# bittremieux/falcon

Measured on AMD Instinct MI355X. Metric: spectra clustered/sec @1/2/4/8 GPU; cosine-kernel HBM GB/s vs roofline, higher is better.
Workload: dtype f32; 1 GPU; one dataset of 1000000 synthetic spectra (1000000 per GPU; charges 2+3; precursor m/z 400-1200), low_dim=400, n_neighbors=64, n_neighbors_ann=128, n_probe=16, eps=0.1, precursor_tol=20ppm, mz_interval=1.0, batch_size=32768; exchange=none, parallelism=1 GPU

## Files before the change

### falcon_amd/csrc/core.hip

```cpp
#include <math.h>
#include <stdarg.h>
#include <stdlib.h>
#include <string.h>
#include "common.h"
#include "hash.h"
#include "scan.h"
#include "ivf.h"
#include <algorithm>

#include <chrono>
namespace fal {
static bool trace_alloc() {
    static int v = -1;
    if (v < 0) {
        const char* e = getenv("FALCON_TRACE_ALLOC");
        v = e && e[0] && e[0] != '0';
    }
    return v == 1;
}
static hipError_t traced_malloc(void** p, size_t bytes, const char* what, int id) {
    if (!trace_alloc()) return hipMalloc(p, bytes);
    const auto t0 = std::chrono::steady_clock::now();
    const hipError_t e = hipMalloc(p, bytes);
    const double ms = std::chrono::duration<double, std::milli>(std::chrono::steady_clock::now() - t0).count();
// ... 128 lines not shown
    if (!arena) FAL_CHECK_HIP(hipHostMalloc((void**)&arena, kArena, hipHostMallocDefault));
    size_t off = (arena_off + 63) & ~(size_t)63;
    if (off + bytes > kArena) {
        FAL_CHECK_HIP(hipStreamSynchronize(stream));
        off = 0;
    }
    memcpy(arena + off, src, bytes);
    FAL_CHECK_HIP(hipMemcpyAsync(dst, arena + off, bytes, hipMemcpyHostToDevice, stream));
    arena_off = off + bytes;
    return FAL_OK;
}

int fal_ctx::stage_begin(int stage, hipEvent_t* stop_out, hipStream_t on) {
    StageTimer& t = timers[stage];
    if (t.used == t.ev.size()) {
        hipEvent_t a, b;
        FAL_CHECK_HIP(hipEventCreate(&a));
        FAL_CHECK_HIP(hipEventCreate(&b));
        t.ev.push_back({a, b});
    }
    FAL_CHECK_HIP(hipEventRecord(t.ev[t.used].first, on ? on : stream));
    *stop_out = t.ev[t.used].second;
    t.used++;
    return FAL_OK;
}

int fal_ctx::stage_end(hipEvent_t stop, hipStream_t on) {
    FAL_CHECK_HIP(hipEventRecord(stop, on ? on : stream));
    return FAL_OK;
}

extern "C" {

int fal_version(void) { return 100; }

const char* fal_last_error(void) { return fal::g_err; }

int fal_device_count(int* count) {
    FAL_REQUIRE(count, FAL_EINVAL, "fal_device_count: NULL");
    int n = 0;
    hipError_t e = hipGetDeviceCount(&n);
    if (e != hipSuccess) n = 0;
    *count = n;
    return FAL_OK;
}

int fal_ctx_create(int device, void* stream, int own_stream, fal_ctx** out) {
    FAL_REQUIRE(out, FAL_EINVAL, "fal_ctx_create: out is NULL");
    *out = nullptr;
    int n = 0;
    if (hipGetDeviceCount(&n) != hipSuccess || n <= 0) {
        fal::set_error("fal_ctx_create: no HIP device visible (this library has no CPU fallback)");
        return FAL_ENODEV;
    }
    FAL_REQUIRE(device >= 0 && device < n, FAL_EINVAL, "fal_ctx_create: device %d out of range [0,%d)", device, n);
    FAL_CHECK_HIP(hipSetDevice(device));
    hipDeviceProp_t prop;
    FAL_CHECK_HIP(hipGetDeviceProperties(&prop, device));
    if (strncmp(prop.gcnArchName, "gfx950", 6) != 0) {
        fal::set_error("fal_ctx_create: device %d is %s; this library is built for gfx950 only", device, prop.gcnArchName);
        return FAL_ENODEV;
    }
    fal_ctx* c = new fal_ctx();
    c->device = device;
    c->num_cus = prop.multiProcessorCount;
    c->persistent_wgs = c->num_cus;
    if (const char* e = getenv("FALCON_PERSISTENT_WGS")) {
        const int v = atoi(e);
        if (v >= 8 && v <= c->num_cus) c->persistent_wgs = v;
    }
    if (!own_stream) {
        c->stream = (hipStream_t)stream;
        c->own_stream = false;
    } else {
        hipError_t e = hipStreamCreateWithFlags(&c->stream, hipStreamNonBlocking);
        if (e != hipSuccess) {
            delete c;
            fal::set_error("hipStreamCreate failed: %s", hipGetErrorString(e));
            return FAL_EHIP;
        }
        c->own_stream = true;
    }
    if (hipHostMalloc((void**)&c->fb_host, 64, hipHostMallocDefault) != hipSuccess ||
        hipMalloc((void**)&c->zero_dev, 64) != hipSuccess || hipMemset(c->zero_dev, 0, 64) != hipSuccess) {
        fal::set_error("fal_ctx_create: cannot allocate the context's counters");
        fal_ctx_destroy(c);
        return FAL_ENOMEM;
    }
    memset(c->fb_host, 0, 64);
    const char* dbg = getenv("FALCON_DEBUG_POISON");
    c->debug_poison = dbg && dbg[0] && dbg[0] != '0';
    *out = c;
    return FAL_OK;
}

int fal_ctx_destroy(fal_ctx* c) {
    if (!c) return FAL_OK;
    (void)hipSetDevice(c->device);
    (void)hipStreamSynchronize(c->stream);
    for (auto& s : c->scratch)
        if (s.ptr) (void)hipFree(s.ptr);
    for (void* p : c->retired) (void)hipFree(p);
    for (auto& b : c->pool) (void)hipFree(b.ptr);
    if (c->pinned) (void)hipHostFree(c->pinned);
    if (c->fb_host) (void)hipHostFree(c->fb_host);
    if (c->zero_dev) (void)hipFree(c->zero_dev);
    if (c->arena) (void)hipHostFree(c->arena);
    for (auto& t : c->timers)
        for (auto& p : t.ev) {
            (void)hipEventDestroy(p.first);
            (void)hipEventDestroy(p.second);
        }
    if (c->own_stream) (void)hipStreamDestroy(c->stream);
    delete c;
    return FAL_OK;
}

int fal_ctx_plan(fal_ctx* c, int64_t n, int low_dim, int k_ann, int n_probe, int64_t batch_size) {
    fal::CallScope _call(c);
    FAL_REQUIRE(c && n >= 0 && low_dim >= 1 && k_ann >= 1 && n_probe >= 1 && batch_size >= 1, FAL_EINVAL, "fal_ctx_plan: bad argument");
    FAL_CHECK_HIP(hipSetDevice(c->device));
    for (const void* k : fal::warm_kernels()) {
        hipFuncAttributes attr;
        FAL_CHECK_HIP(hipFuncGetAttributes(&attr, k));
    }
    if (!c->arena) FAL_CHECK_HIP(hipHostMalloc((void**)&c->arena, (size_t)32u << 20, hipHostMallocDefault));
    if (n == 0) return FAL_OK;
    void* p = nullptr;
    using namespace fal;
    const size_t nn = (size_t)n;
    FAL_TRY(c->reserve(SLOT_SORT, 24 * nn + 4096, &p));
    FAL_TRY(c->reserve(SLOT_SORT2, 12 * nn + 4096, &p));
    {
        const char* e = getenv("FALCON_SIMS_MB");
        size_t cap = (e ? (size_t)atoll(e) : 2048) * 1024 * 1024;
        const double need = 4.0 * (double)nn * (double)std::min<int64_t>(n, std::min<int64_t>(batch_size, 4096));
        if (need < (double)cap) cap = (size_t)need;
        FAL_TRY(c->reserve(SLOT_SIMS, cap + sizeof(float) * kSimsSlack, &p));
    }
    for (int slot : {SLOT_DB, SLOT_DB2, SLOT_TAIL, SLOT_TAIL2, SLOT_FIN, SLOT_FIN2}) FAL_TRY(c->reserve(slot, 8 * nn + 4096, &p));
    for (int slot = 0; slot < fal::kNumSlots; ++slot) c->release(slot);
    return FAL_OK;
}

int fal_ctx_trim(fal_ctx* c) {
    fal::CallScope _call(c);
    FAL_REQUIRE(c, FAL_EINVAL, "fal_ctx_trim: NULL ctx");
    FAL_CHECK_HIP(hipStreamSynchronize(c->stream));
    c->release_retired();
    for (auto& s : c->scratch)
        if (s.ptr) {
            (void)hipFree(s.ptr);
            s.ptr = nullptr;
            s.cap = 0;
        }
    size_t kept = 0;
    for (size_t i = 0; i < c->pool.size(); ++i) {
        if (c->pool[i].used) c->pool[kept++] = c->pool[i];
        else (void)hipFree(c->pool[i].ptr);
    }
    c->pool.resize(kept);
    return FAL_OK;
}

int fal_ctx_sync(fal_ctx* c) {
    fal::CallScope _call(c);
    FAL_REQUIRE(c, FAL_EINVAL, "fal_ctx_sync: NULL ctx");
    FAL_CHECK_HIP(hipStreamSynchronize(c->stream));
    return FAL_OK;
}

int fal_ctx_enable_timing(fal_ctx* c, int on) {
    FAL_REQUIRE(c, FAL_EINVAL, "NULL ctx");
    c->timing = on != 0;
    return FAL_OK;
}

int fal_ctx_counter(fal_ctx* c, int which, int64_t* value) {
    FAL_REQUIRE(c && value && which >= 0 && which < 10, FAL_EINVAL, "fal_ctx_counter: bad argument");
    *value = c->counters[which];
    if (which == 5) *value = c->fb_host ? (int64_t)c->fb_host[0] + (int64_t)c->fb_host[2] : 0;
    return FAL_OK;
}

int fal_ctx_stage_ms(fal_ctx* c, int stage, float* ms, int64_t* launches) {
    fal::CallScope _call(c);
    FAL_REQUIRE(c && ms && stage >= 0 && stage < fal::kNumStages, FAL_EINVAL, "fal_ctx_stage_ms: bad argument");
    FAL_CHECK_HIP(hipStreamSynchronize(c->stream));
    float total = 0.f;
    auto& t = c->timers[stage];
    for (size_t i = 0; i < t.used; ++i) {
        float x = 0.f;
        FAL_CHECK_HIP(hipEventElapsedTime(&x, t.ev[i].first, t.ev[i].second));
        total += x;
    }
    *ms = total;
    if (launches) *launches = (int64_t)t.used;
    return FAL_OK;
}

int fal_get_dim(float min_mz, float max_mz, float bin_size, uint32_t* dim, float* start_dim, float* end_dim) {
    FAL_REQUIRE(dim && start_dim && end_dim, FAL_EINVAL, "fal_get_dim: NULL output");
    FAL_REQUIRE(bin_size > 0.f && max_mz >= min_mz, FAL_EINVAL, "fal_get_dim: need bin_size > 0 and max_mz >= min_mz");
    volatile float s = min_mz - fmodf(min_mz, bin_size);
    volatile float t = max_mz + bin_size;
    volatile float e = t - fmodf(max_mz, bin_size);
    volatile float w = e - s;
    volatile float q = w / bin_size;
    *start_dim = s;
    *end_dim = e;
    *dim = (uint32_t)ceilf(q);
    return FAL_OK;
}

int fal_hash_lookup(uint32_t n_bins, uint32_t low_dim, uint32_t seed, uint32_t* out_table) {
    FAL_REQUIRE(out_table && low_dim > 0, FAL_EINVAL, "fal_hash_lookup: bad argument");
    for (uint32_t i = 0; i < n_bins; ++i) out_table[i] = fal::murmur3_32(i, seed) % low_dim;
    return FAL_OK;
}

}
```

### falcon_amd/csrc/scan.h

```cpp
#pragma once
#include "common.h"
#include "simtile.h"

namespace fal {

enum { EPI_STORE = 0, EPI_ARGMAX = 1 };
enum { MODE_DENSE = 0, MODE_IVF = 1 };

constexpr size_t kSimsSlack = 2048;

struct SelectArgs {
    const float* sims;
    int64_t sims_base;
    int k;
    float* out_sim;
    int32_t* out_idx;
    const DenseJob* jobs;
    int n_jobs;
    int64_t tile_begin;
    const int32_t* tile_job;
    int ids_are_rows;
    int n_probe;
    const int32_t* probes;
    const int64_t* list_off;
    const int64_t* q_sim_off;
    const int32_t* perm;
    const float* f_pmz;
    const float* f_rt;
    double f_tol, f_rt_tol;
    int f_is_da;
    int f_keep;
    int32_t* nb_idx;
    float* nb_dist;
    int32_t* nb_count;
};

bool dense4_supports(int d);
int launch_dense4(fal_ctx* ctx, const float* X, int d, const DenseJob* jobs, const DenseJob* jobs_host, int n_jobs, float* sims,
                  int64_t sims_base);
bool dense4ab_supports(int d);
int launch_dense4ab(fal_ctx* ctx, const float* X, int d, const DenseJob* jobs, const DenseJob* jobs_host, int n_jobs, float* sims,
                    int64_t sims_base);
int launch_dense_tiny4(fal_ctx* ctx, const float* X, int d, const DenseJob* jobs, int n_jobs, float* sims, int64_t sims_base);
int launch_flat_exact_small(fal_ctx* ctx, const float* X, int d, const DenseJob* jobs, int n_jobs, float* sims, int64_t sims_base);
int launch_dense(fal_ctx* ctx, int stage, int epi, const float* Q, const float* Cm, int d, const DenseJob* jobs,
                 int n_jobs, int64_t tile_begin, int64_t n_tiles, float* sims, int64_t sims_base, int32_t* assign,
                 int64_t xcd_list_tiles = 0);
constexpr int kAssignSeg = 2048;
constexpr int kAssignGroup = 128;
constexpr int kAssignMergeLists = 2048;
struct AssignJob {
    int64_t row0;
    int64_t cent0;
    int32_t nrows;
    int32_t ncent;
    int32_t id_base;
    int32_t part0;
};
int launch_assign(fal_ctx* ctx, int stage, const float* X, const float* centroids, int d, const AssignJob* jobs, int64_t n_jobs,
                  int64_t n_wave_jobs, int64_t n, unsigned long long* keys, int32_t* assign);
bool assign16_supports(int d);
int launch_cvt_f16(fal_ctx* ctx, const float* in, void* out, int64_t count);
int launch_assign16(fal_ctx* ctx, int stage, const void* X16, const float* X, const void* C16, const float* Cn, int d,
                    const AssignJob* jobs, int64_t n_single, int64_t n_merge, int64_t n_group, int64_t n_rows, int32_t* assign,
                    uint16_t* ckeys = nullptr, int ckeys_stride = 0, const uint16_t* sp_cols = nullptr,
                    const float* sp_vals = nullptr, int merge_max_lists = 4 * kAssignGroup, int64_t merge_rows = 0);
struct ListScanArgs {
    const float* Xl;
    int d;
    const int64_t* list_off;
    const int64_t* inv_off;
    const int64_t* ltile_off;
    int group_shift;
    const int32_t* inv_q;
    const int64_t* inv_dest;
    int64_t list_begin, list_end;
    int64_t tile_begin, n_tiles_max;
    float* sims;
    int64_t sims_base;
    float* sink;
};
int launch_list_scan(fal_ctx* ctx, const ListScanArgs& a);
int launch_select(fal_ctx* ctx, int stage, int mode, const SelectArgs& a, int64_t n_blocks, hipStream_t on = nullptr);
int launch_scan16(fal_ctx* ctx, int planes, const void* Xs, int d, const DenseJob* jobs, int n_jobs, int64_t list_tiles,
                  float* sims, int64_t sims_base, float* sink);

}
```

### falcon_amd/csrc/scan.hip

```cpp
#include <math.h>
#include <stdlib.h>
#include <string.h>
#include <algorithm>
#include "common.h"
#include "simtile.h"
#include "scan.h"
#include "select.h"
#include "ivf.h"

namespace fal {

template <int DH4, int EPI>
__global__ __launch_bounds__(64, 1) void dense_kernel(
    const float* __restrict__ Q, const float* __restrict__ Cm, int d, const DenseJob* __restrict__ jobs,
    int n_jobs, int64_t tile_begin, int64_t n_tiles, float* __restrict__ sims, int64_t sims_base,
    int32_t* __restrict__ assign, int xcd_lists, int symmetric) {
    DenseJob job;
    int lt;
    int ji = 0;
    if (xcd_lists) {
        if (!find_job_xcd(jobs, n_jobs, blockIdx.x, &ji, &lt)) return;
        job = jobs[ji];
    } else {
        const int64_t per_xcd = (n_tiles + 7) / 8;
// ... 434 lines not shown
}

int launch_flat_exact_small(fal_ctx* ctx, const float* X, int d, const DenseJob* jobs, int n_jobs, float* sims, int64_t sims_base) {
    if (n_jobs <= 0) return FAL_OK;
    StageScope ts(ctx, ST_SCAN);
    hipLaunchKernelGGL(flat_exact_small_kernel, dim3((unsigned)std::min<int64_t>(n_jobs, (int64_t)ctx->num_cus * 16)), dim3(64), 0,
                       ctx->stream, X, d, jobs, n_jobs, sims, sims_base);
    FAL_CHECK_HIP(hipGetLastError());
    return FAL_OK;
}

int launch_dense_tiny4(fal_ctx* ctx, const float* X, int d, const DenseJob* jobs, int n_jobs, float* sims, int64_t sims_base) {
    if (n_jobs <= 0) return FAL_OK;
    const int dh4 = d / 8;
    const size_t lds = (size_t)2 * 32 * (d * 4 + 16);
    int32_t* cursors = nullptr;
    FAL_TRY(ctx->reserve(SLOT_CURSORS, sizeof(int32_t) * 16, (void**)&cursors));
    cursors += 8;
    dim3 grid((unsigned)std::min<int64_t>(ceil_div(n_jobs, 4), ctx->persistent_wgs)), block(256);
    StageScope ts(ctx, ST_SCAN);
    FAL_CHECK_HIP(hipMemsetAsync(cursors, 0, sizeof(int32_t), ctx->stream));
#define FAL_LAUNCH_TINY4(DH4)                                                                                       \
    do {                                                                                                            \
        FAL_CHECK_HIP(hipFuncSetAttribute((const void*)dense_tiny4_kernel<DH4>, hipFuncAttributeMaxDynamicSharedMemorySize, \
                                          (int)lds));                                                               \
        hipLaunchKernelGGL((dense_tiny4_kernel<DH4>), grid, block, lds, ctx->stream, X, d, jobs, n_jobs, sims, sims_base, \
                           cursors);                                                                                \
    } while (0)
    if (dh4 <= 8) FAL_LAUNCH_TINY4(8);
    else if (dh4 <= 16) FAL_LAUNCH_TINY4(16);
    else if (dh4 <= 32) FAL_LAUNCH_TINY4(32);
    else if (dh4 <= 50) FAL_LAUNCH_TINY4(50);
    else {
        set_error("dense_tiny4 supports low_dim <= 400 (got %d)", d);
        return FAL_EUNSUPPORTED;
    }
#undef FAL_LAUNCH_TINY4
    FAL_CHECK_HIP(hipGetLastError());
    return FAL_OK;
}

template <int EPI>
static int launch_dense_t(fal_ctx* ctx, int stage, const float* Q, const float* Cm, int d, const DenseJob* jobs,
                          int n_jobs, int64_t tile_begin, int64_t n_tiles, float* sims, int64_t sims_base,
                          int32_t* assign, int64_t xcd_list_tiles) {
    if (n_tiles <= 0) return FAL_OK;
    const int symmetric = (EPI == EPI_STORE && xcd_list_tiles > 0 && Q == Cm) ? 1 : 0;
    const int dh4 = d / 8;
    const int xcd_lists = xcd_list_tiles > 0;
    const int64_t per_xcd = xcd_lists ? xcd_list_tiles : (n_tiles + 7) / 8;
    FAL_REQUIRE(per_xcd * 8 < (int64_t)INT32_MAX, FAL_EUNSUPPORTED, "too many tiles in one launch");
 dim3 grid((unsigned)(per_xcd * 8)), block(64);
    StageScope ts(ctx, stage);
    StageScope tk(ctx, ST_KERNEL, nullptr, stage == ST_SCAN);
#define FAL_LAUNCH_DENSE(DH4)                                                                              \
    hipLaunchKernelGGL((dense_kernel<DH4, EPI>), grid, block, 0, ctx->stream, Q, Cm, d, jobs, n_jobs,      \
                       tile_begin, n_tiles, sims, sims_base, assign, xcd_lists, symmetric)
    if (dh4 <= 8) FAL_LAUNCH_DENSE(8);
    else if (dh4 <= 16) FAL_LAUNCH_DENSE(16);
    else if (dh4 <= 32) FAL_LAUNCH_DENSE(32);
    else if (dh4 <= 50) FAL_LAUNCH_DENSE(50);
    else if (dh4 <= 64) FAL_LAUNCH_DENSE(64);
    else {
        set_error("float32 scan supports low_dim <= 512 (got %d)", d);
        return FAL_EUNSUPPORTED;
    }
#undef FAL_LAUNCH_DENSE
    FAL_CHECK_HIP(hipGetLastError());
    return FAL_OK;
}

int launch_dense(fal_ctx* ctx, int stage, int epi, const float* Q, const float* Cm, int d, const DenseJob* jobs,
                 int n_jobs, int64_t tile_begin, int64_t n_tiles, float* sims, int64_t sims_base, int32_t* assign,
                 int64_t xcd_list_tiles) {
    if (epi == EPI_STORE)
        return launch_dense_t<EPI_STORE>(ctx, stage, Q, Cm, d, jobs, n_jobs, tile_begin, n_tiles, sims, sims_base,
                                         assign, xcd_list_tiles);
    return launch_dense_t<EPI_ARGMAX>(ctx, stage, Q, Cm, d, jobs, n_jobs, tile_begin, n_tiles, sims, sims_base, assign,
                                      xcd_list_tiles);
}

template <int MODE, bool FUSE>
__global__ __launch_bounds__(64) __attribute__((amdgpu_waves_per_eu(MODE == MODE_DENSE ? 8 : 3, 8))) void select_kernel(SelectArgs a) {
    __shared__ uint32_t sel_u[kSelBuf];
    __shared__ uint32_t sel_id[kSelBuf];
    __shared__ int64_t seg_off[FAL_MAX_N_PROBE + 1];
    __shared__ int64_t seg_src[FAL_MAX_N_PROBE];
    const int lane = threadIdx.x;
    const int k = a.k;
    const unsigned qblock = blockIdx.x;

    SelQuery qy{nullptr, 0, 0};
    int64_t out_row = 0;
    const int64_t t = a.tile_begin + (qblock >> 5);
    const int ql = qblock & 31;
    const DenseJob job = a.jobs[a.tile_job[qblock >> 5]];
    const int lt = (int)(t - job.tile0);
    if (32 * lt + ql >= job.nq) return;
    if (MODE == MODE_DENSE) {
        qy.nc = job.nc;
        qy.row = a.sims + (job.obase - a.sims_base) + (int64_t)(32 * lt + ql) * ((job.nc + 31) & ~31);
        out_row = job.q_row0 + 32 * (int64_t)lt + ql;
        qy.id0 = a.ids_are_rows ? job.c_row0 : 0;
    } else {
        const int64_t p = job.q_row0 + 32 * (int64_t)lt + ql;
        const int np = a.n_probe;
        const int32_t* pr = a.probes + p * np;
        const int64_t lbase = job.c_row0;
        if (lane == 0) {
            int64_t off = 0;
            for (int j = 0; j < np; ++j) {
                const int32_t l = pr[j];
                seg_off[j] = off;
                if (l >= 0) {
                    const int64_t b = a.list_off[lbase + l], e = a.list_off[lbase + l + 1];
                    seg_src[j] = b;
                    off += e - b;
                } else {
                    seg_src[j] = 0;
                }
            }
            seg_off[np] = off;
        }
        __syncthreads();
        qy.nc = seg_off[np];
        qy.row = a.sims + (a.q_sim_off[32 * t + ql] - a.sims_base);
        out_row = a.perm[p];
    }

    int carry;
    if (qy.nc <= 128) carry = select_rounds<MODE, 2>(a, qy, k, lane, sel_u, sel_id, seg_off, seg_src);
    else if (qy.nc <= 256) carry = select_rounds<MODE, 4>(a, qy, k, lane, sel_u, sel_id, seg_off, seg_src);
    else if (qy.nc <= 384) carry = select_rounds<MODE, 6>(a, qy, k, lane, sel_u, sel_id, seg_off, seg_src);
    else if (qy.nc <= 512) carry = select_rounds<MODE, 8>(a, qy, k, lane, sel_u, sel_id, seg_off, seg_src);
    else if (qy.nc <= 768) carry = select_rounds<MODE, 12>(a, qy, k, lane, sel_u, sel_id, seg_off, seg_src);
    else carry = select_rounds<MODE, 16>(a, qy, k, lane, sel_u, sel_id, seg_off, seg_src);

    if constexpr (FUSE) {
        filter_sort_store(a, sel_u, sel_id, sel_u + FAL_MAX_K_ANN, sel_id + FAL_MAX_K_ANN, carry, out_row, lane);
    } else {
        float* osim = a.out_sim + out_row * k;
        int32_t* oidx = a.out_idx + out_row * k;
        if (k <= 64) sort_and_store<1>(sel_u, sel_id, carry, k, lane, osim, oidx);
        else if (k <= 128) sort_and_store<2>(sel_u, sel_id, carry, k, lane, osim, oidx);
        else sort_and_store<4>(sel_u, sel_id, carry, k, lane, osim, oidx);
    }
}

__global__ void tile_job_kernel(const DenseJob* __restrict__ jobs, int n_jobs, int64_t tile_begin, int64_t n_tiles,
                                int32_t* __restrict__ tile_job) {
    const int64_t i = blockIdx.x * (int64_t)blockDim.x + threadIdx.x;
    if (i < n_tiles) tile_job[i] = find_job(jobs, n_jobs, tile_begin + i);
}

int launch_select(fal_ctx* ctx, int stage, int mode, const SelectArgs& a_in, int64_t n_blocks, hipStream_t on) {
    if (n_blocks <= 0) return FAL_OK;
    SelectArgs a = a_in;
    {
        const int64_t n_tiles = n_blocks / 32;
        int32_t* tj = nullptr;
        ctx->release(SLOT_TILEJOB);
        FAL_TRY(ctx->reserve(SLOT_TILEJOB, sizeof(int32_t) * (size_t)std::max<int64_t>(n_tiles, 1 << 16), (void**)&tj));
        hipLaunchKernelGGL(tile_job_kernel, dim3((unsigned)ceil_div(n_tiles, 256)), dim3(256), 0, on ? on : ctx->stream, a.jobs,
                           a.n_jobs, a.tile_begin, n_tiles, tj);
        a.tile_job = tj;
    }
    FAL_REQUIRE(a.k >= 1 && a.k <= FAL_MAX_K_ANN, FAL_EUNSUPPORTED, "k must be in [1, %d]", FAL_MAX_K_ANN);
    FAL_REQUIRE(n_blocks < (int64_t)INT32_MAX, FAL_EUNSUPPORTED, "too many queries in one select launch");
    hipStream_t st = on ? on : ctx->stream;
    StageScope ts(ctx, stage, st);
    const bool fuse = a.nb_idx != nullptr;
    if (fuse) FAL_REQUIRE(a.f_pmz && a.nb_dist && a.f_keep >= 1 && a.f_keep <= FAL_MAX_K_ANN, FAL_EINVAL, "fused filter: bad arguments");
    if (mode == MODE_DENSE && fuse)
        hipLaunchKernelGGL((select_kernel<MODE_DENSE, true>), dim3((unsigned)n_blocks), dim3(64), 0, st, a);
    else if (mode == MODE_DENSE)
        hipLaunchKernelGGL((select_kernel<MODE_DENSE, false>), dim3((unsigned)n_blocks), dim3(64), 0, st, a);
    else if (fuse)
        hipLaunchKernelGGL((select_kernel<MODE_IVF, true>), dim3((unsigned)n_blocks), dim3(64), 0, st, a);
    else
        hipLaunchKernelGGL((select_kernel<MODE_IVF, false>), dim3((unsigned)n_blocks), dim3(64), 0, st, a);
    FAL_CHECK_HIP(hipGetLastError());
    return FAL_OK;
}

}
FAL_WARM_KERNEL(fal::dense4_kernel<50, 0>);
```

### falcon_amd/csrc/search.hip

```cpp
#include <algorithm>
#include <stdlib.h>
#include <string.h>
#include "common.h"
#include "scan.h"
#include "ivf.h"
#include "util.h"
#include "fused.h"
#include "ivf16.h"
#include "coarse16.h"

namespace fal {

template <int NPV>
__global__ void probe_totals_kernel(const int32_t* __restrict__ probes, int np, const DenseJob* __restrict__ jobs,
                                    int n_jobs, int64_t n_tiles, const int64_t* __restrict__ list_off,
                                    int64_t* __restrict__ totals) {
    const int64_t g = blockIdx.x * (int64_t)blockDim.x + threadIdx.x;
    const int64_t t = g >> 5;
    int64_t tot = 0;
    if (t < n_tiles) {
        const DenseJob job = jobs[find_job(jobs, n_jobs, t)];
        const int lt = (int)(t - job.tile0), ql = (int)(g & 31);
        if (32 * lt + ql < job.nq) {
            const int64_t p = job.q_row0 + 32 * (int64_t)lt + ql;
// ... 357 lines not shown
            if (use16) {
                const int x = (int)((cur.j1 - cur.j0) & 7);
                xtile0 = xt16[x];
                xt16[x] += ceil_div(nb, 128);
                cur.jm = cur.js = cur.jk = cur.j1 + 1;
            } else if (use4) {
                xtile0 = 0;
                cur.js = cur.jk = cur.j1 + 1;
            } else if (use1) {
                const int x = (int)((cur.j1 - cur.js) & 7);
                xtile0 = xt1[x];
                xt1[x] += tiles;
                cur.jk = cur.j1 + 1;
            } else {
                const int x = (int)((cur.j1 - cur.jk) & 7);
                xtile0 = xt32[x];
                xt32[x] += tiles;
            }
            flat.push_back({row0, row0, cur.floats, cur.tiles, (int32_t)nb, (int32_t)nb, xtile0});
            cur.tiles += tiles;
            cur.floats += floats;
            cur.j1++;
        }
        close();
    }
    int64_t ivf_tiles = 0, coarse_o = 0;
    int max_n_list = 0;
    for (int64_t b = 0; b < n_buckets; ++b) {
        const int64_t row0 = ivf->bucket_off[b], nb = ivf->bucket_off[b + 1] - row0;
        if (nb == 0 || ivf->n_list[b] == 1) continue;
        const int64_t tiles = ceil_div(nb, 32);
        coarse.push_back({row0, ivf->list_base[b], coarse_o, ivf_tiles, (int32_t)nb, ivf->n_list[b], 0});
        ivf_tiles += tiles;
        coarse_o += tiles * 32 * (((int64_t)ivf->n_list[b] + 31) & ~31ll);
        max_n_list = std::max(max_n_list, ivf->n_list[b]);
    }
    auto make_batches = [&](const std::vector<DenseJob>& jobs, int64_t n_tiles, std::vector<int64_t>& cuts, size_t& need) {
        cuts.assign(1, 0);
        need = 0;
        int64_t used = 0;
        for (const DenseJob& j : jobs) {
            const int64_t tiles = ceil_div(j.nq, 32), per_tile = 32 * (((int64_t)j.nc + 31) & ~31ll);
            for (int64_t t = 0; t < tiles;) {
                int64_t room = ((int64_t)cap - used) / per_tile;
                if (room <= 0 && used > 0) {
                    cuts.push_back(j.tile0 + t);
                    used = 0;
                    continue;
                }
                if (room <= 0) room = 1;
                const int64_t take = std::min(room, tiles - t);
                used += take * per_tile;
                need = std::max(need, (size_t)used);
                t += take;
            }
        }
        if (cuts.back() != n_tiles) cuts.push_back(n_tiles);
    };
    auto obase_of_tile = [&](const std::vector<DenseJob>& jobs, int64_t t) -> int64_t {
        size_t lo = 0, hi = jobs.size() - 1;
        while (lo < hi) {
            size_t mid = (lo + hi + 1) / 2;
            if (jobs[mid].tile0 <= t) lo = mid; else hi = mid - 1;
        }
        return jobs[lo].obase + (t - jobs[lo].tile0) * 32 * (((int64_t)jobs[lo].nc + 31) & ~31ll);
    };

    std::vector<int64_t> coarse_cuts;
    size_t need_coarse = 0;
    if (!coarse.empty()) make_batches(coarse, ivf_tiles, coarse_cuts, need_coarse);

    DenseJob *flat_dev = nullptr, *coarse_dev = nullptr;
    if (!flat.empty()) {
        FAL_TRY(ctx->reserve(SLOT_JOBS, sizeof(DenseJob) * flat.size(), (void**)&flat_dev));
        FAL_TRY(ctx->upload(flat_dev, flat.data(), sizeof(DenseJob) * flat.size()));
    }
    if (!coarse.empty()) {
        FAL_TRY(ctx->reserve(SLOT_JOBS2, sizeof(DenseJob) * coarse.size(), (void**)&coarse_dev));
        FAL_TRY(ctx->upload(coarse_dev, coarse.data(), sizeof(DenseJob) * coarse.size()));
    }
    float* sims = nullptr;
    const size_t sims_floats = std::max(need_flat, need_coarse);
    FAL_TRY(ctx->reserve(SLOT_SIMS, sizeof(float) * (sims_floats + kSimsSlack), (void**)&sims));
    for (size_t bi = 0; bi < flat_batches.size(); ++bi) {
        const FlatBatch& fb = flat_batches[bi];
        float* buf = sims;
        const DenseJob* jb = flat_dev + fb.j0;
        const int nj = (int)(fb.j1 - fb.j0);
        if (fb.jm > fb.j0)
            FAL_TRY(launch_scan16(ctx, ivf->x16_planes, ivf->X16, d, jb, (int)(fb.jm - fb.j0), fb.list_tiles16, buf, 0,
                                  buf + sims_floats));
        if (fb.js > fb.jm)
            FAL_TRY(launch_dense4(ctx, ivf->X, d, flat_dev + fb.jm, flat.data() + fb.jm, (int)(fb.js - fb.jm), buf, 0));
        if (fb.jk > fb.js)
            FAL_TRY(launch_dense(ctx, ST_SCAN, EPI_STORE, ivf->X, ivf->X, d, flat_dev + fb.js, (int)(fb.jk - fb.js), 0, fb.tiles, buf, 0,
                                 nullptr, fb.list_tiles1));
        if (fb.j1 > fb.jk && d > 512)
            FAL_TRY(launch_flat_exact_small(ctx, ivf->X, d, flat_dev + fb.jk, (int)(fb.j1 - fb.jk), buf, 0));
        else if (fb.j1 > fb.jk && have4)
            FAL_TRY(launch_dense_tiny4(ctx, ivf->X, d, flat_dev + fb.jk, (int)(fb.j1 - fb.jk), buf, 0));
        else if (fb.j1 > fb.jk)
            FAL_TRY(launch_dense(ctx, ST_SCAN, EPI_STORE, ivf->X, ivf->X, d, flat_dev + fb.jk, (int)(fb.j1 - fb.jk), 0,
                                 fb.tiles, buf, 0, nullptr, fb.list_tiles32));
        SelectArgs sa{};
        sa.sims = buf; sa.sims_base = 0; sa.k = k_ann; sa.out_sim = sim; sa.out_idx = idx;
        sa.jobs = jb; sa.n_jobs = nj; sa.tile_begin = 0; sa.ids_are_rows = 1;
        set_filter(sa, nf);
        FAL_TRY(launch_select(ctx, ST_SELECT, MODE_DENSE, sa, fb.tiles * 32));
    }
    if (!fused) {
        ctx->counters[0] = 0;
        ctx->counters[4] = 0;
    }
    for (const FlatBatch& fb : flat_batches)
        for (size_t j = fb.j0; j < fb.j1; ++j) {
            const int64_t ch = ceil_div(flat[j].nc, 32);
            ctx->counters[4] += 1024 * (ch * (ch + 1) / 2);
        }
    for (const DenseJob& j : flat) ctx->counters[0] += (int64_t)j.nq * j.nc;
    ctx->counters[7] = ctx->counters[8] = 0;
    if (have4)
        for (const FlatBatch& fb : flat_batches)
            for (size_t j = fb.jk; j < fb.j1; ++j) {
                ctx->counters[7] += (int64_t)flat[j].nq * flat[j].nc;
                ctx->counters[8] += 1024;
            }
    ctx->counters[1] = 0;
    if (!fused) {
        ctx->counters[2] = (int64_t)flat_batches.size();
        ctx->counters[3] = (int64_t)(sizeof(float) * std::max(need_flat, need_coarse));
    }
    if (coarse.empty()) return FAL_OK;
    for (const DenseJob& j : coarse) ctx->counters[1] += (int64_t)j.nq * j.nc;

    const int np = std::min(n_probe, max_n_list);
    int32_t* probes = nullptr;
    float* probe_sim = nullptr;
    int64_t *totals = nullptr, *q_sim_off = nullptr;
    FAL_TRY(ctx->reserve(SLOT_PROBES, sizeof(int32_t) * (size_t)ivf->n * np, (void**)&probes));
    FAL_TRY(ctx->reserve(SLOT_PROBE_SIM, sizeof(float) * (size_t)ivf->n * np, (void**)&probe_sim));
    const int64_t n_slots = ivf_tiles * 32;
    FAL_TRY(ctx->reserve(SLOT_QOFF, sizeof(int64_t) * (size_t)(n_slots + 1), (void**)&q_sim_off));
    FAL_TRY(ctx->reserve(SLOT_MISC, sizeof(int64_t) * (size_t)(n_slots + 2), (void**)&totals));
    FAL_CHECK_HIP(hipMemsetAsync(totals, 0, sizeof(int64_t) * (size_t)(n_slots + 2), st));
    const bool from_keys = ivf->ckeys != nullptr && ivf->X != nullptr &&
                           (ivf->ckeys_stride <= 512 || (ivf->ckeys_stride <= 2048 && ivf->sp_cols != nullptr));
    if (from_keys) {
        Coarse16Args ca{ivf->ckeys, ivf->ckeys_stride, ivf->X, ivf->centroids, d, coarse_dev, (int)coarse.size(), ivf_tiles, nullptr,
                        ivf->perm, np, probes};
        ca.sp_cols = ivf->sp_cols;
        ca.sp_vals = ivf->sp_vals;
        FAL_TRY(launch_coarse16(ctx, ca));
    }
    if (!from_keys) FAL_TRY(ivf_ensure_xl(ctx, ivf));
    for (size_t bi = 0; !from_keys && bi + 1 < coarse_cuts.size(); ++bi) {
        const int64_t t0 = coarse_cuts[bi], t1 = coarse_cuts[bi + 1];
        const int64_t base = obase_of_tile(coarse, t0);
        FAL_TRY(launch_dense(ctx, ST_COARSE, EPI_STORE, ivf->Xl, ivf->centroids, d, coarse_dev, (int)coarse.size(), t0,
                             t1 - t0, sims, base, nullptr));
        SelectArgs sa{};
        sa.sims = sims; sa.sims_base = base; sa.k = np; sa.out_sim = probe_sim; sa.out_idx = probes;
        sa.jobs = coarse_dev; sa.n_jobs = (int)coarse.size(); sa.tile_begin = t0; sa.ids_are_rows = 0;
        FAL_TRY(launch_select(ctx, ST_COARSE, MODE_DENSE, sa, (t1 - t0) * 32));
    }
    const bool fused_totals = max_n_list <= 4096;
    if (!fused_totals) {
        StageScope ts(ctx, ST_COARSE);
        const dim3 tg((unsigned)ceil_div(n_slots, 256));
        if (np == 16)
            hipLaunchKernelGGL(probe_totals_kernel<4>, tg, dim3(256), 0, st, probes, np, coarse_dev, (int)coarse.size(), ivf_tiles,
                               ivf->list_off, totals);
        else if (np == 32)
            hipLaunchKernelGGL(probe_totals_kernel<8>, tg, dim3(256), 0, st, probes, np, coarse_dev, (int)coarse.size(), ivf_tiles,
                               ivf->list_off, totals);
        else
            hipLaunchKernelGGL(probe_totals_kernel<0>, tg, dim3(256), 0, st, probes, np, coarse_dev, (int)coarse.size(), ivf_tiles,
                               ivf->list_off, totals);
        FAL_TRY(device_scan_i64(ctx, totals, n_slots, q_sim_off, SLOT_MISC2));
    }
    const int group_shift = 7;
    const int64_t TL = ivf->total_lists;
    const int64_t n_pairs_max = ivf->n * (int64_t)np;
    int32_t *cnt = nullptr, *inv_q = nullptr;
    int64_t *inv_off = nullptr, *inv_dest = nullptr;
    FAL_TRY(ctx->reserve(SLOT_INVCNT, sizeof(int32_t) * (size_t)(3 * TL + 3) + sizeof(int64_t) * (size_t)(2 * TL + 4), (void**)&inv_off));
    int64_t* ltile_off = inv_off + (TL + 2);
    cnt = reinterpret_cast<int32_t*>(ltile_off + (TL + 2));
    int32_t* cursor = cnt + (TL + 1);
    int32_t* ltiles = cursor + (TL + 1);
    const bool want_rows = nf && ivf->X16pre && ivf->pos_of_row && max_n_list <= 16384;
    FAL_TRY(ctx->reserve(SLOT_INV, (sizeof(int64_t) + (want_rows ? 2 : 1) * sizeof(int32_t)) * (size_t)n_pairs_max + 1024, (void**)&inv_dest));
    inv_q = reinterpret_cast<int32_t*>(inv_dest + n_pairs_max);
// ... 197 lines not shown
```

### falcon_amd/csrc/select.h

```cpp
#pragma once
#include <math.h>
#include "common.h"
#include "simtile.h"
#include "scan.h"

namespace fal {

__device__ __forceinline__ int wave_count(bool p) { return __popcll(__ballot(p)); }

struct SelQuery {
    const float* row;
    int64_t nc;
    int64_t id0;
};

template <int MODE, int R>
__device__ __forceinline__ int select_round(const SelectArgs& a, const SelQuery& qy, int k, int lane, int fresh,
                                            uint32_t* sel_u, uint32_t* sel_id, const int64_t* seg_off,
                                            const int64_t* seg_src) {
    uint32_t u[R];
    const float* rl = qy.row + lane;
    float fv[R];
#pragma unroll
    for (int i = 0; i < R; ++i) fv[i] = rl[i * 64];
    const uint32_t id_lane = (uint32_t)(qy.id0 + lane);
    auto real_id = [&](int64_t pp) -> uint32_t {
        pp = min<int64_t>(pp, qy.nc - 1);
        int lo = 0, hi = a.n_probe - 1;
        while (lo < hi) {
            const int mid = (lo + hi + 1) >> 1;
            if (seg_off[mid] <= pp) lo = mid; else hi = mid - 1;
        }
        return (uint32_t)a.perm[seg_src[lo] + (pp - seg_off[lo])];
    };
    auto id_of = [&](int i) -> uint32_t {
        return MODE == MODE_DENSE ? id_lane + (uint32_t)(i * 64) : real_id(i * 64 + lane);
    };
#pragma unroll
    for (int i = 0; i < R; ++i) u[i] = (i * 64 + lane < fresh) ? max(f32_sortable(fv[i]), 1u) : 0u;
    const int m = fresh;

    uint32_t T = 1, I = 0xFFFFFFFFu;
    if (m > k) {
        uint32_t mn = 0xFFFFFFFFu, mx = 0u;
#pragma unroll
        for (int i = 0; i < R; ++i) {
            mn = min(mn, u[i] ? u[i] : 0xFFFFFFFFu);
            mx = max(mx, u[i]);
        }
        mn = wave_min_u32(mn);
        mx = wave_max_u32(mx);
        int shift = 32 - __clz((int)(mn ^ mx));
        if (mn == mx) shift = 0;
        uint32_t prefix = shift >= 32 ? 0u : (mx >> shift) << shift;
        int kk = k, eq = m;
        bool exact = false;
        uint32_t* hist = sel_u;
        while (shift > 0 && !exact) {
            const int wbits = min(8, shift);
            const int hi = shift;
            shift -= wbits;
            const uint32_t dmask = (1u << wbits) - 1u;
            const uint32_t himask = hi >= 32 ? 0u : ~0u << hi;
            *reinterpret_cast<uint4*>(hist + 4 * lane) = make_uint4(0u, 0u, 0u, 0u);
            wave_lds_sync();
#pragma unroll
            for (int i = 0; i < R; ++i)
                if (u[i] != 0u && (u[i] & himask) == prefix)
                    __hip_atomic_fetch_add(&hist[(u[i] >> shift) & dmask], 1u, __ATOMIC_RELAXED, __HIP_MEMORY_SCOPE_WORKGROUP);
            wave_lds_sync();
            const uint4 cv = *reinterpret_cast<const uint4*>(hist + 4 * lane);
            const int c[4] = {(int)cv.x, (int)cv.y, (int)cv.z, (int)cv.w};
            const int own = c[0] + c[1] + c[2] + c[3];
            const int pre = wave_prefix_sum(own);
            const int suf = __builtin_amdgcn_readlane(pre, 63) - pre + own;
            const int L = 63 - __clzll((unsigned long long)__ballot(suf >= kk));
            int acc = suf - own, bin = 4 * lane, cj = c[0];
#pragma unroll
            for (int j = 3; j >= 0; --j) {
                if (acc + c[j] >= kk) { bin = 4 * lane + j; cj = c[j]; break; }
                acc += c[j];
            }
            acc = __builtin_amdgcn_readlane(acc, L);
            bin = __builtin_amdgcn_readlane(bin, L);
            cj = __builtin_amdgcn_readlane(cj, L);
            kk -= acc;
            prefix |= (uint32_t)bin << shift;
            exact = cj == kk;
            eq = cj;
            wave_lds_sync();
        }
        T = prefix;
        if (!exact) {
            const int need = kk;
            if (eq > need) {
                uint32_t lo = 0;
                for (int bit = 31; bit >= 0; --bit) {
// ... 251 lines not shown
            osim[e] = valid ? sortable_f32(hi[r]) : -INFINITY;
            oidx[e] = valid ? (int32_t)~lo[r] : -1;
        }
    }
}

template <int SIZE>
__device__ __forceinline__ void sort_small(uint32_t& hi, uint32_t& lo, int lane) {
    uint32_t h[1] = {hi}, l[1] = {lo};
    bitonic_build<1, SIZE>(h, l, lane);
    hi = h[0];
    lo = l[0];
}

template <int E>
__device__ __forceinline__ void sort_and_store_nb(const uint32_t* f_u, const uint32_t* f_lo, int c, int keep, int lane,
                                                  int32_t* __restrict__ onb, float* __restrict__ odist) {
    uint32_t hi[E], lo[E];
#pragma unroll
    for (int r = 0; r < E; ++r) {
        const int e = lane * E + r;
        hi[r] = e < c ? f_u[e] : 0u;
        lo[r] = e < c ? f_lo[e] : 0u;
    }
    if constexpr (E == 1) {
        if (c <= 2) sort_small<2>(hi[0], lo[0], lane);
        else if (c <= 4) sort_small<4>(hi[0], lo[0], lane);
        else if (c <= 8) sort_small<8>(hi[0], lo[0], lane);
        else if (c <= 16) sort_small<16>(hi[0], lo[0], lane);
        else if (c <= 32) sort_small<32>(hi[0], lo[0], lane);
        else sort_small<64>(hi[0], lo[0], lane);
    } else {
        bitonic_build<E, 64 * E>(hi, lo, lane);
    }
#pragma unroll
    for (int r = 0; r < E; ++r) {
        const int e = lane * E + r;
        if (e < keep) {
            const bool valid = e < c;
            onb[e] = valid ? (int32_t)~lo[r] : -1;
            odist[e] = valid ? fminf(fmaxf(1.0f - sortable_f32(hi[r]), 0.f), 1.f) : INFINITY;
        }
    }
    for (int e = 64 * E + lane; e < keep; e += 64) {
        onb[e] = -1;
        odist[e] = INFINITY;
    }
}

__device__ __forceinline__ void rank_or_sort_and_store_nb(const uint2* keys, int c, int keep, int lane, int32_t* __restrict__ onb,
                                                          float* __restrict__ odist) {
    const uint2 mine = lane < c ? keys[lane] : make_uint2(0u, 0u);
    if (c <= 16) {
        const unsigned long long me = ((unsigned long long)mine.y << 32) | mine.x;
        int rank = 0;
        for (int j = 0; j < c; ++j) {
            const uint2 kj = keys[j];
            rank += ((((unsigned long long)kj.y << 32) | kj.x) > me) ? 1 : 0;
        }
        if (lane < c && rank < keep) {
            onb[rank] = (int32_t)~mine.x;
            odist[rank] = fminf(fmaxf(1.0f - sortable_f32(mine.y), 0.f), 1.f);
        }
        for (int e = c + lane; e < keep; e += 64) {
            onb[e] = -1;
            odist[e] = INFINITY;
        }
        return;
    }
    uint32_t hi = mine.y, lo = mine.x;
    if (c <= 32) sort_small<32>(hi, lo, lane);
    else sort_small<64>(hi, lo, lane);
    if (lane < keep) {
        const bool valid = lane < c;
        onb[lane] = valid ? (int32_t)~lo : -1;
        odist[lane] = valid ? fminf(fmaxf(1.0f - sortable_f32(hi), 0.f), 1.f) : INFINITY;
    }
    for (int e = 64 + lane; e < keep; e += 64) {
        onb[e] = -1;
        odist[e] = INFINITY;
    }
}

__device__ __forceinline__ void filter_sort_store(const SelectArgs& a, const uint32_t* sel_u, const uint32_t* sel_id,
                                                  uint32_t* f_u, uint32_t* f_lo, int carry, int64_t row, int lane) {
    const float qmz = a.f_pmz[row];
    const bool use_rt = a.f_rt != nullptr && a.f_rt_tol >= 0.0;
    const float qrt = use_rt ? a.f_rt[row] : 0.f;
    int c = 0;
    for (int e0 = 0; e0 < carry; e0 += 64) {
        const int e = e0 + lane;
        bool ok = false;
        uint32_t u = 0, id = 0;
        if (e < carry) {
            u = sel_u[e];
            id = sel_id[e];
            if ((int64_t)id != row) {
                const float nmz = a.f_pmz[id];
                const float diff = qmz - nmz;
                const double md = a.f_is_da ? (double)diff : (double)(diff / nmz) * 1e6;
                ok = fabs(md) <= a.f_tol;
                if (ok && use_rt) ok = fabs((double)(qrt - a.f_rt[id])) <= a.f_rt_tol;
            }
        }
        const uint64_t mask = __ballot(ok);
        if (ok) {
            const int w = c + __popcll(mask & ((1ull << lane) - 1ull));
            f_u[w] = u;
            f_lo[w] = ~id;
        }
        c += __popcll(mask);
    }
    __syncthreads();
    int32_t* onb = a.nb_idx + row * a.f_keep;
    float* odist = a.nb_dist + row * a.f_keep;
    if (a.nb_count && lane == 0) a.nb_count[row] = min(c, a.f_keep);
    if (c <= 64) sort_and_store_nb<1>(f_u, f_lo, c, a.f_keep, lane, onb, odist);
    else if (c <= 128) sort_and_store_nb<2>(f_u, f_lo, c, a.f_keep, lane, onb, odist);
    else sort_and_store_nb<4>(f_u, f_lo, c, a.f_keep, lane, onb, odist);
}


}
```

Before: 185.4 million spectra/s.

## Add precursor-window fast path to fused dense select using sorted m/z

Adds a kernel that checks whether precursor m/z values are sorted and positive, writing the result into a device flag. When the flag is clear, the fused dense select kernel looks only at the 128 neighbours around each query's position that pass the precursor tolerance. It finds their rank among all candidates with a radix-histogram k-th-key search, then sorts and stores only those survivors, instead of running full top-k rounds followed by filtering. A query whose window runs past the 128-entry bounds falls back to the old path and increments a counter, which is exposed through counter 9. The aim is to cut select work for dense buckets, at the cost of an extra pass over the m/z array and more complex select code.

```diff
diff --git a/falcon_amd/csrc/core.hip b/falcon_amd/csrc/core.hip
--- a/falcon_amd/csrc/core.hip
+++ b/falcon_amd/csrc/core.hip
@@ -234,7 +234,7 @@
         c->own_stream = true;
     }
     if (hipHostMalloc((void**)&c->fb_host, 64, hipHostMallocDefault) != hipSuccess ||
-        hipMalloc((void**)&c->zero_dev, 64) != hipSuccess || hipMemset(c->zero_dev, 0, 64) != hipSuccess) {
+        hipMalloc((void**)&c->zero_dev, 128) != hipSuccess || hipMemset(c->zero_dev, 0, 128) != hipSuccess) {
         fal::set_error("fal_ctx_create: cannot allocate the context's counters");
         fal_ctx_destroy(c);
         return FAL_ENOMEM;
@@ -332,6 +332,7 @@
     FAL_REQUIRE(c && value && which >= 0 && which < 10, FAL_EINVAL, "fal_ctx_counter: bad argument");
     *value = c->counters[which];
     if (which == 5) *value = c->fb_host ? (int64_t)c->fb_host[0] + (int64_t)c->fb_host[2] : 0;
+    if (which == 9) *value = !c->fb_host ? 0 : c->fb_host[3] ? -1 : (int64_t)c->fb_host[4];
     return FAL_OK;
 }
 
diff --git a/falcon_amd/csrc/scan.h b/falcon_amd/csrc/scan.h
--- a/falcon_amd/csrc/scan.h
+++ b/falcon_amd/csrc/scan.h
@@ -33,6 +33,7 @@
     int32_t* nb_idx;
     float* nb_dist;
     int32_t* nb_count;
+    int32_t* win_state;
 };
 
 bool dense4_supports(int d);
@@ -82,6 +83,7 @@
 };
 int launch_list_scan(fal_ctx* ctx, const ListScanArgs& a);
 int launch_select(fal_ctx* ctx, int stage, int mode, const SelectArgs& a, int64_t n_blocks, hipStream_t on = nullptr);
+int launch_pmz_order(fal_ctx* ctx, const float* pmz, int64_t n, int32_t* state);
 int launch_scan16(fal_ctx* ctx, int planes, const void* Xs, int d, const DenseJob* jobs, int n_jobs, int64_t list_tiles,
                   float* sims, int64_t sims_base, float* sink);
 
diff --git a/falcon_amd/csrc/scan.hip b/falcon_amd/csrc/scan.hip
--- a/falcon_amd/csrc/scan.hip
+++ b/falcon_amd/csrc/scan.hip
@@ -540,8 +540,8 @@
 
 template <int MODE, bool FUSE>
 __global__ __launch_bounds__(64) __attribute__((amdgpu_waves_per_eu(MODE == MODE_DENSE ? 8 : 3, 8))) void select_kernel(SelectArgs a) {
-    __shared__ uint32_t sel_u[kSelBuf];
-    __shared__ uint32_t sel_id[kSelBuf];
+    __shared__ __align__(16) uint32_t sel_u[kSelBuf];
+    __shared__ __align__(16) uint32_t sel_id[kSelBuf];
     __shared__ int64_t seg_off[FAL_MAX_N_PROBE + 1];
     __shared__ int64_t seg_src[FAL_MAX_N_PROBE];
     const int lane = threadIdx.x;
@@ -586,6 +586,23 @@
         out_row = a.perm[p];
     }
 
+    if constexpr (MODE == MODE_DENSE && FUSE) {
+        if (a.win_state && a.ids_are_rows && job.q_row0 == job.c_row0 && job.nq == job.nc && qy.nc <= 1024 && a.win_state[0] == 0) {
+            const int p = 32 * lt + ql;
+            bool ok_a = false, ok_b = false;
+            if (window_probe(a, a.f_pmz + job.c_row0, job.nc, p, job.c_row0, lane, ok_a, ok_b)) {
+                if (qy.nc <= 128) window_select<2>(a, qy, k, lane, p, ok_a, ok_b, out_row, sel_u, sel_id);
+                else if (qy.nc <= 256) window_select<4>(a, qy, k, lane, p, ok_a, ok_b, out_row, sel_u, sel_id);
+                else if (qy.nc <= 384) window_select<6>(a, qy, k, lane, p, ok_a, ok_b, out_row, sel_u, sel_id);
+                else if (qy.nc <= 512) window_select<8>(a, qy, k, lane, p, ok_a, ok_b, out_row, sel_u, sel_id);
+                else if (qy.nc <= 768) window_select<12>(a, qy, k, lane, p, ok_a, ok_b, out_row, sel_u, sel_id);
+                else window_select<16>(a, qy, k, lane, p, ok_a, ok_b, out_row, sel_u, sel_id);
+                return;
+            }
+            if (lane == 0) atomicAdd(a.win_state + 1, 1);
+        }
+    }
+
     int carry;
     if (qy.nc <= 128) carry = select_rounds<MODE, 2>(a, qy, k, lane, sel_u, sel_id, seg_off, seg_src);
     else if (qy.nc <= 256) carry = select_rounds<MODE, 4>(a, qy, k, lane, sel_u, sel_id, seg_off, seg_src);
@@ -609,6 +626,22 @@
                                 int32_t* __restrict__ tile_job) {
     const int64_t i = blockIdx.x * (int64_t)blockDim.x + threadIdx.x;
     if (i < n_tiles) tile_job[i] = find_job(jobs, n_jobs, tile_begin + i);
+}
+
+__global__ void pmz_order_kernel(const float* __restrict__ pmz, int64_t n, int32_t* __restrict__ state) {
+    const int64_t i = blockIdx.x * (int64_t)blockDim.x + threadIdx.x;
+    if (i >= n) return;
+    const float v = pmz[i];
+    if (!(v > 0.f && v < INFINITY) || (i + 1 < n && !(v <= pmz[i + 1]))) state[0] = 1;
+}
+
+int launch_pmz_order(fal_ctx* ctx, const float* pmz, int64_t n, int32_t* state) {
+    FAL_CHECK_HIP(hipMemsetAsync(state, 0, 2 * sizeof(int32_t), ctx->stream));
+    if (n <= 0) return FAL_OK;
+    StageScope ts(ctx, ST_SELECT);
+    hipLaunchKernelGGL(pmz_order_kernel, dim3((unsigned)ceil_div(n, 256)), dim3(256), 0, ctx->stream, pmz, n, state);
+    FAL_CHECK_HIP(hipGetLastError());
+    return FAL_OK;
 }
 
 int launch_select(fal_ctx* ctx, int stage, int mode, const SelectArgs& a_in, int64_t n_blocks, hipStream_t on) {
diff --git a/falcon_amd/csrc/search.hip b/falcon_amd/csrc/search.hip
--- a/falcon_amd/csrc/search.hip
+++ b/falcon_amd/csrc/search.hip
@@ -463,6 +463,11 @@
     float* sims = nullptr;
     const size_t sims_floats = std::max(need_flat, need_coarse);
     FAL_TRY(ctx->reserve(SLOT_SIMS, sizeof(float) * (sims_floats + kSimsSlack), (void**)&sims));
+    int32_t* win_state = nullptr;
+    if (nf && !flat_batches.empty()) {
+        win_state = ctx->zero_dev + 16;
+        FAL_TRY(launch_pmz_order(ctx, nf->pmz, ivf->n, win_state));
+    }
     for (size_t bi = 0; bi < flat_batches.size(); ++bi) {
         const FlatBatch& fb = flat_batches[bi];
         float* buf = sims;
@@ -487,8 +492,10 @@
         sa.sims = buf; sa.sims_base = 0; sa.k = k_ann; sa.out_sim = sim; sa.out_idx = idx;
         sa.jobs = jb; sa.n_jobs = nj; sa.tile_begin = 0; sa.ids_are_rows = 1;
         set_filter(sa, nf);
+        sa.win_state = win_state;
         FAL_TRY(launch_select(ctx, ST_SELECT, MODE_DENSE, sa, fb.tiles * 32));
     }
+    FAL_CHECK_HIP(hipMemcpyAsync(ctx->fb_host + 3, win_state ? win_state : ctx->zero_dev, 2 * sizeof(int32_t), hipMemcpyDeviceToHost, st));
     if (!fused) {
         ctx->counters[0] = 0;
         ctx->counters[4] = 0;
diff --git a/falcon_amd/csrc/select.h b/falcon_amd/csrc/select.h
--- a/falcon_amd/csrc/select.h
+++ b/falcon_amd/csrc/select.h
@@ -13,6 +13,79 @@
     int64_t nc;
     int64_t id0;
 };
+
+template <int R, class IdOf>
+__device__ __forceinline__ void kth_key(const uint32_t (&u)[R], int m, int k, int lane, uint32_t* hist, IdOf id_of, uint32_t wa,
+                                        uint32_t wb, uint32_t& T, uint32_t& I, int& low) {
+    uint32_t mn = 0xFFFFFFFFu, mx = 0u;
+#pragma unroll
+    for (int i = 0; i < R; ++i) {
+        mn = min(mn, u[i] ? u[i] : 0xFFFFFFFFu);
+        mx = max(mx, u[i]);
+    }
+    mn = wave_min_u32(mn);
+    mx = wave_max_u32(mx);
+    int shift = 32 - __clz((int)(mn ^ mx));
+    if (mn == mx) shift = 0;
+    uint32_t prefix = shift >= 32 ? 0u : (mx >> shift) << shift;
+    int kk = k, eq = m;
+    bool exact = false, settled = false;
+    while (shift > 0 && !exact) {
+        const int wbits = min(8, shift);
+        const int hi = shift;
+        shift -= wbits;
+        const uint32_t dmask = (1u << wbits) - 1u;
+        const uint32_t himask = hi >= 32 ? 0u : ~0u << hi;
+        *reinterpret_cast<uint4*>(hist + 4 * lane) = make_uint4(0u, 0u, 0u, 0u);
+        wave_lds_sync();
+#pragma unroll
+        for (int i = 0; i < R; ++i)
+            if (u[i] != 0u && (u[i] & himask) == prefix)
+                __hip_atomic_fetch_add(&hist[(u[i] >> shift) & dmask], 1u, __ATOMIC_RELAXED, __HIP_MEMORY_SCOPE_WORKGROUP);
+        wave_lds_sync();
+        const uint4 cv = *reinterpret_cast<const uint4*>(hist + 4 * lane);
+        const int c[4] = {(int)cv.x, (int)cv.y, (int)cv.z, (int)cv.w};
+        const int own = c[0] + c[1] + c[2] + c[3];
+        const int pre = wave_prefix_sum(own);
+        const int suf = __builtin_amdgcn_readlane(pre, 63) - pre + own;
+        const int L = 63 - __clzll((unsigned long long)__ballot(suf >= kk));
+        int acc = suf - own, bin = 4 * lane, cj = c[0];
+#pragma unroll
+        for (int j = 3; j >= 0; --j) {
+            if (acc + c[j] >= kk) { bin = 4 * lane + j; cj = c[j]; break; }
+            acc += c[j];
+        }
+        acc = __builtin_amdgcn_readlane(acc, L);
+        bin = __builtin_amdgcn_readlane(bin, L);
+        cj = __builtin_amdgcn_readlane(cj, L);
+        kk -= acc;
+        prefix |= (uint32_t)bin << shift;
+        exact = cj == kk;
+        eq = cj;
+        wave_lds_sync();
+        const uint32_t lomask = ~0u << shift;
+        if (!exact && !__ballot((wa != 0u && (wa & lomask) == prefix) || (wb != 0u && (wb & lomask) == prefix))) {
+            settled = true;
+            break;
+        }
+    }
+    T = prefix;
+    low = shift;
+    if (!exact && !settled) {
+        const int need = kk;
+        if (eq > need) {
+            uint32_t lo = 0;
+            for (int bit = 31; bit >= 0; --bit) {
+                const uint32_t c = lo | (1u << bit);
+                int cnt = 0;
+#pragma unroll
+                for (int i = 0; i < R; ++i) cnt += wave_count(u[i] == T && id_of(i) < c);
+                if (cnt < need) lo = c;
+            }
+            I = lo;
+        }
+    }
+}
 
 template <int MODE, int R>
 __device__ __forceinline__ int select_round(const SelectArgs& a, const SelQuery& qy, int k, int lane, int fresh,
@@ -430,6 +503,14 @@
     }
 }
 
+__device__ __forceinline__ bool within_tolerance(const SelectArgs& a, float qmz, float qrt, bool use_rt, float nmz, int64_t id) {
+    const float diff = qmz - nmz;
+    const double md = a.f_is_da ? (double)diff : (double)(diff / nmz) * 1e6;
+    bool ok = fabs(md) <= a.f_tol;
+    if (ok && use_rt) ok = fabs((double)(qrt - a.f_rt[id])) <= a.f_rt_tol;
+    return ok;
+}
+
 __device__ __forceinline__ void filter_sort_store(const SelectArgs& a, const uint32_t* sel_u, const uint32_t* sel_id,
                                                   uint32_t* f_u, uint32_t* f_lo, int carry, int64_t row, int lane) {
     const float qmz = a.f_pmz[row];
@@ -443,13 +524,7 @@
         if (e < carry) {
             u = sel_u[e];
             id = sel_id[e];
-            if ((int64_t)id != row) {
-                const float nmz = a.f_pmz[id];
-                const float diff = qmz - nmz;
-                const double md = a.f_is_da ? (double)diff : (double)(diff / nmz) * 1e6;
-                ok = fabs(md) <= a.f_tol;
-                if (ok && use_rt) ok = fabs((double)(qrt - a.f_rt[id])) <= a.f_rt_tol;
-            }
+            if ((int64_t)id != row) ok = within_tolerance(a, qmz, qrt, use_rt, a.f_pmz[id], id);
         }
         const uint64_t mask = __ballot(ok);
         if (ok) {
@@ -469,4 +544,74 @@
 }
 
 
-}
+__device__ __forceinline__ bool window_probe(const SelectArgs& a, const float* pm, int n_b, int p, int64_t row0, int lane,
+                                             bool& ok_a, bool& ok_b) {
+    const int pa = p - 64 + lane, pb = p + lane;
+    const bool va = pa >= 0, vb = pb < n_b;
+    const float na = va ? pm[pa] : 0.f, nb = vb ? pm[pb] : 0.f;
+    const float qmz = pm[p];
+    const double q = (double)qmz, w = a.f_tol * (1.0 + 0x1p-20);
+    bool ma, mb;
+    if (a.f_is_da) {
+        ma = va && (double)na + w >= q && (double)na - w <= q;
+        mb = vb && (double)nb + w >= q && (double)nb - w <= q;
+    } else {
+        const double up = 1.0 + w * 1e-6, dn = 1.0 - w * 1e-6;
+        ma = va && (double)na * up >= q && (double)na * dn <= q;
+        mb = vb && (double)nb * up >= q && (double)nb * dn <= q;
+    }
+    const uint64_t run_a = __ballot(ma), run_b = __ballot(mb);
+    if (((run_a & 1ull) && p - 64 > 0) || ((run_b >> 63) && p + 63 < n_b - 1)) return false;
+    const bool use_rt = a.f_rt != nullptr && a.f_rt_tol >= 0.0;
+    const float qrt = use_rt ? a.f_rt[row0 + p] : 0.f;
+    ok_a = ma && within_tolerance(a, qmz, qrt, use_rt, na, row0 + pa);
+    ok_b = mb && lane != 0 && within_tolerance(a, qmz, qrt, use_rt, nb, row0 + pb);
+    return true;
+}
+
+template <int R>
+__device__ __forceinline__ void window_select(const SelectArgs& a, const SelQuery& qy, int k, int lane, int p, bool ok_a, bool ok_b,
+                                              int64_t row, uint32_t* sel_u, uint32_t* sel_id) {
+    const int m = (int)qy.nc;
+    const float fa = ok_a ? qy.row[p - 64 + lane] : 0.f, fb = ok_b ? qy.row[p + lane] : 0.f;
+    const uint32_t wa = ok_a ? max(f32_sortable(fa), 1u) : 0u, wb = ok_b ? max(f32_sortable(fb), 1u) : 0u;
+    const uint32_t id_a = (uint32_t)(qy.id0 + p - 64 + lane), id_b = (uint32_t)(qy.id0 + p + lane);
+    uint32_t T = 1, I = 0xFFFFFFFFu;
+    int low = 0;
+    if (m > k && __ballot(ok_a || ok_b)) {
+        uint32_t u[R];
+        const float* rl = qy.row + lane;
+        float fv[R];
+#pragma unroll
+        for (int i = 0; i < R; ++i) fv[i] = rl[i * 64];
+#pragma unroll
+        for (int i = 0; i < R; ++i) u[i] = (i * 64 + lane < m) ? max(f32_sortable(fv[i]), 1u) : 0u;
+        const uint32_t id_lane = (uint32_t)(qy.id0 + lane);
+        kth_key<R>(u, m, k, lane, sel_u, [&](int i) -> uint32_t { return id_lane + (uint32_t)(i * 64); }, wa, wb, T, I, low);
+    }
+    const uint32_t himask = low >= 32 ? 0u : ~0u << low;
+    const bool in_a = wa != 0u && ((wa & himask) > T || ((wa & himask) == T && (I == 0xFFFFFFFFu || id_a <= I)));
+    const bool in_b = wb != 0u && ((wb & himask) > T || ((wb & himask) == T && (I == 0xFFFFFFFFu || id_b <= I)));
+    const uint64_t mask_a = __ballot(in_a), mask_b = __ballot(in_b), below = (1ull << lane) - 1ull;
+    const int c_a = __popcll(mask_a), c = c_a + __popcll(mask_b);
+    uint2* keys = reinterpret_cast<uint2*>(sel_u);
+    if (in_a) keys[__popcll(mask_a & below)] = make_uint2(~id_a, wa);
+    if (in_b) keys[c_a + __popcll(mask_b & below)] = make_uint2(~id_b, wb);
+    __syncthreads();
+    int32_t* onb = a.nb_idx + row * a.f_keep;
+    float* odist = a.nb_dist + row * a.f_keep;
+    if (a.nb_count && lane == 0) a.nb_count[row] = min(c, a.f_keep);
+    if (c <= 64) {
+        rank_or_sort_and_store_nb(keys, c, a.f_keep, lane, onb, odist);
+    } else {
+        uint32_t* f_u = sel_id, * f_lo = sel_id + 128;
+        for (int e = lane; e < c; e += 64) {
+            f_u[e] = keys[e].y;
+            f_lo[e] = keys[e].x;
+        }
+        __syncthreads();
+        sort_and_store_nb<2>(f_u, f_lo, c, a.f_keep, lane, onb, odist);
+    }
+}
+
+}
```

After: 180.8 million spectra/s. 0.975x the previous value.
